# FibonacciDude/ContrastiveProsthetics

Measured on AMD Instinct MI355X. Metric: sEMG windows/sec contrastive step, 12-ch Ninapro, 1/2/4/8 MI355X, higher is better.
Workload: dtype bf16; 1 GPU; synthetic 12-ch sEMG, 41-class one-hot, batch 4096 groups/GPU (167936 windows/GPU/step), stock BN (--no_adabn), dp_emg=0.0635, d_e=16, random-init weights; global_batch_groups=4096, parallelism=dp1, loss=reference per-group loss, tile_schedule=static

## Files before the change

contrastiveprosthetics_amd/_lib.py:

```python
from __future__ import annotations

import ctypes as C
import os

_HERE = os.path.dirname(os.path.abspath(__file__))
LIB_PATH = os.environ.get("CPNATIVE_LIB") or os.path.join(_HERE, "libcpnative.so")

CP_F32, CP_BF16, CP_FP8 = 0, 1, 2
FP8_STATE_BYTES = 1024
CP_TASKS, CP_EMG_DIM, CP_D_E, CP_N_BN, CP_N_FC = 41, 12, 16, 9, 7

_fp = C.c_void_p


class cp_params(C.Structure):
    _fields_ = [
        ("conv1_w", _fp), ("conv1_b", _fp), ("conv2_w", _fp), ("conv2_b", _fp),
        ("fc_w", _fp * CP_N_FC), ("fc_b", _fp * CP_N_FC),
        ("bn_g", _fp * CP_N_BN), ("bn_b", _fp * CP_N_BN),
        ("last_w", _fp), ("easy_w", _fp), ("easy_b", _fp),
    ]


class cp_bn_buffers(C.Structure):
    _fields_ = [("running_mean", _fp * CP_N_BN), ("running_var", _fp * CP_N_BN)]


ALLREDUCE_FN = C.CFUNCTYPE(C.c_int, C.c_void_p, C.c_void_p, C.c_int64, C.c_void_p)

OPTIONS = {"unfused_bn_bwd": 1, "unpaired_wgrad": 2, "fp8_bridge": 4, "no_small": 8, "fp8_head_f32": 16}
CP_TILES_STATIC, CP_TILES_DYNAMIC = 0, 1


class cp_forward_record(C.Structure):
    _fields_ = [("n_windows", C.c_int64), ("path", C.c_int32), ("backwards", C.c_int32), ("transposed", C.c_int32),
                ("pad", C.c_int32), ("join_event", C.c_void_p)]


class cp_config(C.Structure):
    _fields_ = [
        ("n_windows", C.c_int64), ("dtype", C.c_int32), ("adabn", C.c_int32),
        ("training", C.c_int32), ("step_state_lo", C.c_uint32),
        ("dp_emg", C.c_float), ("bn_momentum", C.c_float), ("bn_eps", C.c_float), ("step_state_hi", C.c_uint32),
        ("seed", C.c_uint64), ("step", C.c_uint64),
        ("options", C.c_uint32), ("tile_schedule", C.c_int32),
# ... 327 lines not shown
```

contrastiveprosthetics_amd/csrc/common.cuh:

```cuda
#pragma once
#include <hip/hip_runtime.h>
#include <stdint.h>
#include <type_traits>
#include <utility>

typedef uint16_t bf16_t;
typedef __attribute__((ext_vector_type(8))) short s16x8;
typedef __attribute__((ext_vector_type(4))) short s16x4;
typedef __attribute__((ext_vector_type(4))) float f32x4;
typedef __attribute__((ext_vector_type(16))) float f32x16;

#define CP_WAVE 64

template <class F, int... I>
__device__ __forceinline__ void static_for_impl(F&& f, std::integer_sequence<int, I...>) { (f(std::integral_constant<int, I>{}), ...); }
template <int N, class F>
__device__ __forceinline__ void static_for(F&& f) { static_for_impl(f, std::make_integer_sequence<int, N>{}); }


__device__ __forceinline__ float bf2f(bf16_t h) { return __uint_as_float(((uint32_t)h) << 16); }
__device__ __forceinline__ bf16_t f2bf(float f) {
    return __builtin_bit_cast(bf16_t, (__bf16)f);
}
typedef __bf16 bf16x2_t __attribute__((ext_vector_type(2)));
// ... 175 lines not shown
#pragma unroll
    for (int o = 32; o > 0; o >>= 1) v += __shfl_xor(v, o, 64);
    return v;
}
__device__ __forceinline__ float wave_max(float v) {
#pragma unroll
    for (int o = 32; o > 0; o >>= 1) v = fmaxf(v, __shfl_xor(v, o, 64));
    return v;
}
__device__ __forceinline__ double wave_sum_d(double v) {
#pragma unroll
    for (int o = 32; o > 0; o >>= 1) v += __shfl_xor(v, o, 64);
    return v;
}

static inline int cdiv(int64_t a, int64_t b) { return (int)((a + b - 1) / b); }
```

contrastiveprosthetics_amd/csrc/conv_kernels.cuh:

```cuda
#pragma once
#include <type_traits>
#include "common.cuh"
#include "gemm_tn.cuh"

#define CONV_WPB 16
#define CONV_ROWS (CONV_WPB * 12)
#define CONV_IMG_ROWS (CONV_WPB * 14)

struct ConvArgs {
    const float* x;
    const float* w1;
    const float* b1;
    const float* stats1;
    const void* wc;
    const float* bias2;
    const void* gin;
    const int* gin_exp;
    const float* coef;
    void* out;
    uint8_t* out8;
    const int* out_exp;
    uint32_t* out_amax;
    float* partials;
    int64_t n_windows;
// ... 582 lines not shown

    for (int i = tid; i < 64 * (192 / EPC); i += 256) {
        const int row = i / (192 / EPC), ch = i % (192 / EPC);
        *(uint4*)(Wl + row * WPITCH + ch * 16) = *(const uint4*)((const T*)a.wc + row * 192 + ch * EPC);
    }
    for (int i = tid; i < 2 * CONV_WPB * 16; i += 256) (&xpad[0][0])[i] = 0.f;
    const int ch1 = ft * 32 + r;
    const float w0 = a.w1[ch1 * 9 + 3], w1 = a.w1[ch1 * 9 + 4], w2 = a.w1[ch1 * 9 + 5], b1 = a.b1[ch1];
    float ca, cb, cz;
    if constexpr (ROWS) {
        __shared__ float ca_s[64], cb_s[64], cz_s[64];
        conv_bn_bwd_coef(a.rows1, a.rows1_nr, 1, a.stats1, (double)a.n_windows * 12, ca_s, cb_s, cz_s, (double (*)[4][64])smem, blockIdx.x == 0,
                         a.dgamma1, a.dbeta1);
        ca = ca_s[ch1]; cb = cb_s[ch1]; cz = cz_s[ch1];
        __syncthreads();
    } else {
        ca = a.coef[ch1]; cb = a.coef[64 + ch1]; cz = a.coef[128 + ch1];
    }
    float d0 = 0.f, d1 = 0.f, d2 = 0.f, d3 = 0.f;

    auto load_x = [&](int64_t strip) {
        const int64_t i = strip * (CONV_WPB * 12) + tid;
        return (tid < CONV_WPB * 12 && strip < nstrips && i < total_rows) ? a.x[i] : 0.f;
    };
    const int xslot = (tid / 12) * 16 + 1 + tid % 12;
    constexpr int NITG = CONV_IMG_ROWS / RPP;
    GV pg[NITG];
    float gd = 1.f;
    if constexpr (G8) gd = f8_exp2i(-*a.gin_exp);
    auto prefetch_g = [&](int64_t strip) {
// ... 100 lines not shown
```

contrastiveprosthetics_amd/csrc/encoder_api.cuh:

```cuda
static const int kLayerC[CP_N_BN] = {64, 64, 512, 512, 512, 512, 512, 512, 512};
static inline int fcK(int i) { return i == 0 ? 768 : 512; }
static inline size_t align256(size_t x) { return (x + 255) & ~(size_t)255; }

struct WS {
    size_t act[CP_N_BN];
    size_t u[4];
    size_t gbuf[2];
    size_t dz;
    size_t partials;
    size_t partials2;
    size_t stats[CP_N_BN];
    size_t coef;
    size_t wc2_f, wc2_d;
    size_t wfc[CP_N_FC], bfc[CP_N_FC], wfc_t[CP_N_FC];
    size_t wlast, blast, wlast_t, dzsum;
    size_t slabs;
    size_t praw;
    size_t head_part;
    size_t sm_acc;
    size_t sync_loc, sync_glob;
    size_t gkeep[3], slabs_b;
    size_t f8state, act8[CP_N_BN], u8[3], wfc8[CP_N_FC], wsc8[CP_N_FC];
    size_t g8[2], wfc8t[CP_N_FC], wsc8t[CP_N_FC];
    size_t total;
// ... 160 lines not shown
static inline int grid_rows(int64_t rows, int rows_per_block, int cap) {
    int64_t g = (rows + rows_per_block - 1) / rows_per_block;
    return (int)(g > cap ? cap : (g < 1 ? 1 : g));
}

template <typename T> static inline int fc_bm() { return sizeof(T) == 2 ? 256 : 128; }
template <typename T, int EPI>
static inline hipError_t launch_fc_gemm(const GemmNTArgs& a, hipStream_t st, int* stat_rows = nullptr, bool dyn_schedule = false) {
    if (stat_rows) *stat_rows = (int)((a.M + fc_bm<T>() - 1) / fc_bm<T>());
    if constexpr (sizeof(T) == 2) {
        const bool dyn = dyn_schedule, ws_ok = !dyn;
        if (EPI == EPI_FWD && a.K == WS_K && a.lda == WS_K && a.relu && ws_ok) return launch_gemm_ws(a, st, stat_rows);
        if (EPI == EPI_FWD && a.K == WSK_K && a.lda == WSK_K && a.F == 512 && a.relu && ws_ok) return launch_gemm_ws16n(a, st, stat_rows);
        if (EPI == EPI_FWD || (a.R == nullptr && a.dp_thresh == 0)) return launch_gemm_nt256p<EPI>(a, st, stat_rows, dyn);
        if (EPI == EPI_DGRAD && a.R != nullptr && a.K == WS_K && a.lda == WS_K && ws_ok) return launch_gemm_wsd_bn(a, st, stat_rows);
        if constexpr (EPI == EPI_DGRAD)
            return a.coef ? launch_gemm_nt256p<EPI_DGRAD_BN>(a, st, stat_rows, dyn) : launch_gemm_nt256p<EPI_DGRAD_ST>(a, st, stat_rows, dyn);
        return hipErrorInvalidValue;
    } else {
        return launch_gemm_nt<T, 128, 128, ALOAD_PLAIN, EPI>(a, st);
    }
}

template <typename T>
static inline int conv_grid(int64_t n_windows) {
    const int64_t strips = (n_windows + CONV_WPB - 1) / CONV_WPB;
    const int64_t cap = sizeof(T) == 2 ? 512 : 256;
    return (int)(strips < cap ? strips : cap);
}

// ... 482 lines not shown

static int bwd_finalize(const Pass& ctx, cp_params* g, const float* pp, int nr, double count, int l, int C, int nfold, const char* what) {
    const cp_config* c = ctx.cfg;
    const float* local = nullptr;
    if (c->stats_allreduce) {
        if (int e = sync_row(c, pp, nr, 2 * C * nfold, ctx.base, ctx.w, ctx.st, &pp, &local)) return e;
        nr = 1;
        count *= c->stats_world;
    }
    hipLaunchKernelGGL(bn_bwd_finalize_kernel, dim3(FIN_GRID(C)), dim3(FIN_THREADS), 0, ctx.st, pp, nr, count, ctx.stats(l), ctx.coef, g->bn_g[l],
                       g->bn_b[l], C, nfold, local);
    CKL(what);
    return 0;
}

static int bias_grad_from_rows(const Pass& ctx, int rows, int C, float* db, const char* what) {
    const float* pp = ctx.pre(rows, C);
    hipLaunchKernelGGL(colsum_finalize_kernel, dim3(FIN_GRID(C)), dim3(FIN_THREADS), 0, ctx.st, pp, rows, C, db);
    CKL(what);
    return 0;
}

template <typename T>
static int proj_dz_sums(const ProjLaunch& ctx, const T* dz, float* dzsum) {
    using D = DT<T>;
    const int gb = grid_rows(ctx.N, 256 / (CP_D_E / D::EPC), 64);
    hipLaunchKernelGGL((colsum_kernel<T>), dim3(gb), dim3(256), 256 * D::EPC * 4, ctx.st, dz, ctx.partials, ctx.N, 64, CP_D_E);
    hipLaunchKernelGGL(colsum_finalize_kernel, dim3(FIN_GRID(CP_D_E)), dim3(FIN_THREADS), 0, ctx.st, ctx.partials, gb, CP_D_E, dzsum);
    CKL("colsum(dz)");
    return 0;
// ... 194 lines not shown
    if (!small && gcol_rows <= 0) {
        if (int e = launch_conv2_gcols<T>(ctx.conv(), cur, &gcol_rows)) return e;
    }
    ConvArgs ca{};
    ca.x = x; ca.w1 = p->conv1_w; ca.b1 = p->conv1_b; ca.stats1 = nullptr; ca.gin = cur; ca.n_windows = N;
    if (small) {
        float* gcols3 = (float*)(base + w.praw);
        ca.bn2_rows = partials; ca.bn2_nr = stat_rows; ca.r2 = ctx.act<T>(1); ca.stats2 = ctx.stats(1);
        ca.dgamma2 = g->bn_g[1]; ca.dbeta2 = g->bn_b[1]; ca.gcols3 = gcols3;
        if (int e = conv2_wgrad<T>(ctx.conv(), p, g, ca, true, false, nullptr, 0, gcols3, g->conv2_b)) return e;
        if (int e = tap_gradient(c, 1, cur, N, 768, sizeof(T), st)) return e;
    } else {
        ca.gin_exp = g8 ? (const int*)&g8->e[F8_T_GRAD + 1] : nullptr;
        if (int e = conv2_wgrad<T>(ctx.conv(), p, g, ca, false, g8 != nullptr, partials, gcol_rows, nullptr, nullptr)) return e;
        ProfScope ps(CP_K_BN_BWD, st);
        if (int e = bwd_finalize(ctx, g, ctx.rows2(), CONV2_FINISH_ROWS, (double)R12, 0, 64, 1, "bn_bwd_finalize_kernel(conv1)")) return e;
        ca.coef = ctx.coef;
    }
    int grid_d = 0;
    ca.wc = base + w.wc2_d;
    if (c->grad_tap) {
        ca.out = nxt; ca.partials = partials;
        if (g8) ca.gin = (unsigned char*)c->grad_tap + (size_t)N * 768 * 2;
        if (int e = launch_conv2_dgrad<T>(ctx.conv(), ca, &grid_d)) return e;
        ca.gin = cur;
        if (int e = tap_gradient(c, 0, nxt, N, 768, sizeof(T), st)) return e;
    }
    {
        ca.out = nullptr; ca.partials = partials;
        if (small) {
            ca.stats1 = ctx.stats(0); ca.rows1 = ctx.rows2(); ca.rows1_nr = CONV2_FINISH_ROWS;
            ca.dgamma1 = g->bn_g[0]; ca.dbeta1 = g->bn_b[0];
// ... 98 lines not shown
    if (int e = aux.fork()) return e;
    {
        ProfScope ps(CP_K_PROJ_BWD, st);
        const ProjLaunch pl = ctx.proj();
        const float *s = nullptr, *t = nullptr;
        float* dzsum = (float*)(base + w.dzsum);
        if (!drop) {
            s = ctx.scale(8); t = ctx.shift(8);
            if (int e = proj_dz_sums<T>(pl, dz, dzsum)) return e;
        }
        ProjDrop dp{};
        if (drop) set_dropout(dp, ctx, 8);
        const hipStream_t sw = aux.s();
        int S;
        const bool proj_alg = fuse_ok && drop && sizeof(T) == 2;
        if (proj_alg) {
            if constexpr (sizeof(T) == 2) {
                if (int e = launch_proj_wgrad_onepass(pl, (const bf16_t*)dz, ctx.act<T>(8), nullptr, slabs, dp, ctx.scale(8), ctx.shift(8), p->last_w, g->last_w, &S)) return e;
            }
        } else {
            if (int e = launch_proj_wgrad_tn<T>(pl, sw, dz, ctx.act<T>(8), nullptr, aux.on ? (float*)(base + w.slabs_b) : slabs, ctx.scale(8), ctx.shift(8), dp,
                                                s, t, dzsum, g->last_w, drop ? (float*)nullptr : praw, &S)) return e;
        }
        if (!drop) {
            if (int e = proj_sums_from_wgrad(pl, p->last_w, praw, dzsum)) return e;
            stat_rows = 1;
        }
        GemmNTArgs a{};
        a.A = dz; a.lda = 64; a.M = N; a.K = 64;
        a.W = base + w.wlast_t; a.F = 512;
        a.C = cur; a.ldc = 512; a.R = drop ? ctx.act<T>(8) : nullptr; a.ldr = 512; a.partials = partials;
        if (drop) set_dropout(a, ctx, 8);
        int drows = 0;
        if (fuse_ok && !drop) {
            if (int e = bwd_finalize(ctx, g, partials, stat_rows, (double)N, 8, 512, 1, "bn_bwd_finalize_kernel(fc7, fused)")) return e;
            a.R = ctx.act<T>(8); a.coef = coef; a.coef_mod = 512;
            CK((launch_fc_gemm<T, EPI_DGRAD>(a, st, &drows, dyn_tiles(c))));
            if (int e = bias_grad_from_rows(ctx, drows, 512, g->fc_b[6], "colsum_finalize_kernel(fc7, fused)")) return e;
            bn_done = true;
        } else if (proj_alg) {
            if (int e = bwd_finalize(ctx, g, partials, PROJ_FINISH_ROWS, (double)N, 8, 512, 1, "bn_bwd_finalize_kernel(fc7, projection)")) return e;
            a.coef = coef; a.coef_mod = 512;
            CK(launch_proj_dgrad(a, st, &drows));
            if (int e = bias_grad_from_rows(ctx, drows, 512, g->fc_b[6], "colsum_finalize_kernel(fc7, projection)")) return e;
            bn_done = true;
        } else {
            CK((launch_fc_gemm<T, EPI_DGRAD>(a, st, &drows, dyn_tiles(c))));
            if (drop) stat_rows = drows;
        }
    }
    struct { const T* X; const T* Y; int i; } pend{};
    bool pending = false;
    for (int L = 8; L >= 2; --L) {
        const int i = L - 2, Lp = L - 1, K = fcK(i);
        if (!bn_done) {
            ProfScope ps(CP_K_BN_BWD, st);
            int nr = stat_rows;
            const float* pp = ctx.pre(nr, 2 * 512);
            if (int e = bwd_finalize(ctx, g, pp, nr, (double)N, L, 512, 1, "bn_bwd_finalize_kernel")) return e;
            const int gb = grid_rows(N, 256 / (512 / D::EPC), CAP_BRB16);
            hipLaunchKernelGGL((bn_relu_bwd_kernel<T>), dim3(gb), dim3(256), 256 * D::EPC * 4, st, cur, ctx.act<T>(L), coef, partials, N, 512);
            if (int e = bias_grad_from_rows(ctx, gb, 512, g->fc_b[i], "bn_relu_bwd_kernel")) return e;
        }
        if (int e = tap_gradient(c, L, cur, N, 512, sizeof(T), st)) return e;
        const bool in_drop = drop && Lp >= 5;
        const T* Y = in_drop ? (const T*)(base + w.u[Lp - 5]) : ctx.act<T>(Lp);
        const float* s = in_drop ? nullptr : ctx.scale(Lp);
        const float* t = in_drop ? nullptr : ctx.shift(Lp);
        int S;
        WgradPlace pl;
        if (int e = place_wgrad(ctx, aux, in_drop, i, sizeof(T) == 2 && !opt(c, CP_OPT_UNPAIRED_WGRAD), &pl)) return e;
        if (pl.defer) {
            pend.X = cur; pend.Y = Y; pend.i = i;
            pending = true;
        } else if constexpr (sizeof(T) == 2) {
            GemmTN256Args ta{};
            ta.X = (const bf16_t*)cur; ta.ldx = 512; ta.Y = (const bf16_t*)Y; ta.ldy = K; ta.slabs = pl.slabs; ta.M = N; ta.P = 512; ta.Q = K;
            if (pending) { ta.X2 = (const bf16_t*)pend.X; ta.Y2 = (const bf16_t*)pend.Y; ta.slabs2 = pl.slabs + (size_t)32 * 512 * 512; }
            split_rows(N, pending ? 32 : (K == 512 ? 64 : 40), &S, &ta.rows_per_split);
            ta.splits = S;
            ProfScope ps(CP_K_FC_WGRAD, pl.sw);
            CK(launch_gemm_tn256(ta, pl.sw));
        } else {
            GemmTNArgs ta{};
            ta.X = cur; ta.ldx = 512; ta.Y = Y; ta.ldy = K; ta.slabs = slabs; ta.M = N; ta.P = 512; ta.Q = K;
            split_rows(N, 32, &S, &ta.rows_per_split);
            ProfScope ps(CP_K_FC_WGRAD, st);
            CK((launch_gemm_tn<T, 128, 128, YLOAD_PLAIN>(ta, S, st)));
        }
        if (!pl.defer) {
            ProfScope ps(CP_K_REDUCE_SLABS, pl.sw);
            if (pending) {
                hipLaunchKernelGGL(reduce_slabs_kernel<float>, dim3(512), dim3(256), 0, pl.sw, pl.slabs + (size_t)32 * 512 * 512, S, 512, 512, 512,
                                   (const float*)nullptr, (const float*)nullptr, g->fc_b[pend.i], g->fc_w[pend.i], 0, (float*)nullptr);
                CKL("reduce_slabs(fc, deferred)");
                pending = false;
            }
            hipLaunchKernelGGL(reduce_slabs_kernel<float>, dim3(512), dim3(256), 0, pl.sw, pl.slabs, S, 512, K, 512, s, t, g->fc_b[i], g->fc_w[i],
                               i == 0 ? 1 : 0, in_drop ? (float*)nullptr : praw);
            CKL("reduce_slabs(fc)");
            if (!in_drop) {
                hipLaunchKernelGGL(bn_bwd_sums_from_wgrad_kernel, dim3(K / 64, kSumSlices), dim3(256), 0, st, praw, p->fc_w[i],
                                   g->fc_b[i], partials, 512, K, i == 0 ? 1 : 0);
                CKL("bn_bwd_sums_from_wgrad_kernel");
            }
        }
        stat_rows = in_drop ? tiles_n : kSumSlices;
        GemmNTArgs a{};
        a.A = cur; a.lda = 512; a.M = N; a.K = 512;
        a.W = base + w.wfc_t[i]; a.F = K;
        a.C = nxt; a.ldc = K; a.R = in_drop ? ctx.act<T>(Lp) : nullptr; a.ldr = K; a.partials = partials;
        if (in_drop) set_dropout(a, ctx, Lp);
        bn_done = false;
        if (fuse_ok && !in_drop) {
            const int Cp = kLayerC[Lp], nfold = K / Cp;
            {
                ProfScope ps(CP_K_BN_BWD, st);
                int nr = stat_rows;
                const float* pp = ctx.pre(nr, 2 * K);
                if (int e = bwd_finalize(ctx, g, pp, nr, (double)N * nfold, Lp, Cp, nfold, "bn_bwd_finalize_kernel(fused)")) return e;
            }
            a.R = ctx.act<T>(Lp); a.coef = coef; a.coef_mod = Cp;
            int drows = 0;
            {
                ProfScope ps(CP_K_FC_DGRAD_BN, st);
                CK((launch_fc_gemm<T, EPI_DGRAD>(a, st, &drows, dyn_tiles(c))));
            }
            if (Lp == 1) gcol_rows = drows;
            {
                ProfScope ps(CP_K_BN_BWD, st);
                if (int e = bias_grad_from_rows(ctx, drows * nfold, Cp, Lp >= 2 ? g->fc_b[i - 1] : g->conv2_b, "colsum_finalize_kernel(fused)")) return e;
            }
            bn_done = true;
        } else {
            ProfScope ps(in_drop ? CP_K_FC_DGRAD_STATS : CP_K_FC_DGRAD, st);
// ... 272 lines not shown
```

contrastiveprosthetics_amd/csrc/gemm_nt.cuh:

```cuda
#pragma once
#include "common.cuh"

enum { ALOAD_PLAIN = 0, ALOAD_CONV = 1,
       ALOAD_BNDROP = 2,
       ALOAD_F8 = 3,
       ALOAD_BNDROP_F8 = 4 };
enum { EPI_FWD = 0, EPI_DGRAD = 1, EPI_PLAIN_F32 = 2,
       EPI_DGRAD_BN = 3,
       EPI_DGRAD_ST = 4 };

struct GemmNTArgs {
    const void* A;
    const void* W;
    void* C;
    const float* bias;
    const void* R;
    float* partials;
    const float* coef;
    int coef_mod;
    const float* a_scale;
    const float* a_shift;
    const int* a_exp;
    int64_t M;
    int lda, ldc, ldr;
    int K, F;
    int relu;
    int f_valid;
    int pad0;
    uint32_t dp_thresh, dp_key;
    const uint32_t* dp_salt;
    float dp_inv_keep;
    int* sched;
};

template <typename T, int BM, int BN, int ALOAD, int EPI>
__global__ __launch_bounds__(256) void gemm_nt_kernel(GemmNTArgs a) {
    using D = DT<T>;
    constexpr int EPC = D::EPC;
    constexpr int BK = D::BK;
    constexpr int WAVES_F = (BN >= 128) ? 2 : 1;
    constexpr int WAVES_S = 4 / WAVES_F;
    constexpr int WS_T = BM / (WAVES_S * 32);
    constexpr int WF_T = BN / (WAVES_F * 32);
    constexpr int A_BYTES = BM * 128, W_BYTES = BN * 128;
    constexpr int C_PITCH = BN * (int)sizeof(T) + 16;
    constexpr int STAGE_BYTES = 2 * (A_BYTES + W_BYTES);
    constexpr int C_BYTES = (EPI == EPI_PLAIN_F32) ? 0 : BM * C_PITCH;
// ... 225 lines not shown
```

contrastiveprosthetics_amd/csrc/gemm_ws.cuh:

```cuda
#pragma once
#include "gemm_nt256p.cuh"

#define WS_K 512

template <typename V4, typename RSRC>
__device__ __forceinline__ void store_b128_settled(const V4& c, RSRC rsrc, uint32_t voff, uint32_t soff, int ) {
    __builtin_amdgcn_raw_buffer_store_b128(c, rsrc, voff, soff, 0);
    asm volatile("s_nop 1" :: "v"(c));
}

typedef __attribute__((ext_vector_type(4))) unsigned int u32x4_t;
__device__ __forceinline__ void bufl16_lds(const u32x4_t& rsrc, uint32_t voff, uint32_t soff_uniform, uint32_t lds_dst_uniform) {
    uint32_t keep;
    asm volatile("s_mov_b32 %0, m0\n\ts_mov_b32 m0, %4\n\ts_nop 0\n\tbuffer_load_dwordx4 %1, %2, %3 offen lds\n\ts_mov_b32 m0, %0"
                 : "=&s"(keep)
                 : "v"(voff), "s"(rsrc), "s"(soff_uniform), "s"(lds_dst_uniform)
                 : "memory");
}

typedef __attribute__((ext_vector_type(4))) float f32x4_t;
#define WS16_RT 48
#define WS16_ST (WS16_RT / 16)
#define WS16_TILE_BYTES (WS16_RT * WS_K * 2)
struct Ws16Acc {
// ... 359 lines not shown
    if (stat_rows) *stat_rows = (int)(tiles < workers ? tiles : workers);
    if (a.partials != nullptr) hipLaunchKernelGGL(gemm_ws16n_kernel<true>, dim3(256), dim3(256), 0, st, a);
    else hipLaunchKernelGGL(gemm_ws16n_kernel<false>, dim3(256), dim3(256), 0, st, a);
    return hipGetLastError();
}


#define WSD16_RT 32

template <int MODE>
__global__ __launch_bounds__(256, 1) void gemm_wsd16_kernel(GemmNTArgs a) {
    constexpr bool STATS = MODE == 1;
    constexpr int RT = WSD16_RT, TILE_BYTES = RT * WS_K * 2, R_BYTES = RT * 128;
    constexpr int K = WS_K, KB = K / 32, RPW = RT / 4, ST = RT / 16;
    constexpr int R_OFF = 2 * TILE_BYTES, COEF_OFF = R_OFF + 4 * 2 * R_BYTES;
    __shared__ __attribute__((aligned(16))) unsigned char smem[COEF_OFF];

    const int tid = threadIdx.x, lane = tid & 63;
    const int wave = __builtin_amdgcn_readfirstlane(tid >> 6);
    const int s16 = lane & 15, q4 = lane >> 4;
    const int xcd = blockIdx.x & 7, j = blockIdx.x >> 3;
    const int nfb = a.F >> 8;
    const int nwk = 32 / nfb;
    const int fb = j % nfb, wkr = j / nfb;
    const int64_t tiles = (a.M + RT - 1) / RT;
    const int first = wkr * 8 + xcd, stride = nwk * 8;
    const int ntile = (wkr < nwk && first < tiles) ? (int)((tiles - first + stride - 1) / stride) : 0;
    if (ntile == 0) return;
    const uint32_t dkey = (STATS && a.dp_thresh != 0) ? (a.dp_salt ? (a.dp_key ^ *a.dp_salt) : a.dp_key) : 0u;
    const int f0 = fb * 256 + wave * 64;
    float4 cfa[STATS ? 1 : 4], cfb[STATS ? 1 : 4], cfz[STATS ? 1 : 4];
    if constexpr (!STATS) {
#pragma unroll
        for (int ft = 0; ft < 4; ++ft) {
            float v[3][4];
#pragma unroll
            for (int c = 0; c < 3; ++c)
#pragma unroll
                for (int e = 0; e < 4; ++e) v[c][e] = a.coef[c * a.coef_mod + (f0 + ft * 16 + 4 * (lane >> 4) + e) % a.coef_mod];
            cfa[ft] = make_float4(v[0][0], v[0][1], v[0][2], v[0][3]);
            cfb[ft] = make_float4(v[1][0], v[1][1], v[1][2], v[1][3]);
            cfz[ft] = make_float4(v[2][0], v[2][1], v[2][2], v[2][3]);
        }
    }

    s16x8 wreg[4][KB];
    {
        const bf16_t* Wg = (const bf16_t*)a.W + (int64_t)(f0 + s16) * K + 8 * q4;
#pragma unroll
        for (int ft = 0; ft < 4; ++ft)
#pragma unroll
            for (int kb = 0; kb < KB; ++kb)
                asm volatile("global_load_dwordx4 %0, %1, off" : "=a"(wreg[ft][kb]) : "v"(Wg + (int64_t)ft * 16 * K + kb * 32) : "memory");
        asm volatile("s_waitcnt vmcnt(0)" ::: "memory");
#pragma unroll
        for (int ft = 0; ft < 4; ++ft)
#pragma unroll
            for (int kb = 0; kb < KB; kb += 8)
                asm volatile("s_waitcnt vmcnt(0)" : "+a"(wreg[ft][kb]), "+a"(wreg[ft][kb + 1]), "+a"(wreg[ft][kb + 2]), "+a"(wreg[ft][kb + 3]),
                             "+a"(wreg[ft][kb + 4]), "+a"(wreg[ft][kb + 5]), "+a"(wreg[ft][kb + 6]), "+a"(wreg[ft][kb + 7]));
// ... 168 lines not shown
    constexpr int COEF_OFF = 4 * 2 * R_BYTES;
    __shared__ __attribute__((aligned(16))) unsigned char smem[COEF_OFF + 3 * 256 * 4];
    float* coef_s = (float*)(smem + COEF_OFF);

    const int tid = threadIdx.x, lane = tid & 63;
    const int wave = __builtin_amdgcn_readfirstlane(tid >> 6);
    const int s16 = lane & 15, q4 = lane >> 4;
    const int xcd = blockIdx.x & 7, j = blockIdx.x >> 3;
    const int nfb = a.F >> 8;
    const int nwk = (gridDim.x >> 3) / nfb;
    const int fb = j % nfb, wkr = j / nfb;
    const int64_t tiles = (a.M + RT - 1) / RT;
    const int first = wkr * 8 + xcd, stride = nwk * 8;
    const int ntile = (wkr < nwk && first < tiles) ? (int)((tiles - first + stride - 1) / stride) : 0;
    if (ntile == 0) return;
    for (int q = tid; q < 3 * 256; q += 256) {
        const int c = q >> 8, f = fb * 256 + (q & 255);
        coef_s[q] = a.coef[c * a.coef_mod + f % a.coef_mod];
    }
    __syncthreads();
    const int f0 = fb * 256 + wave * 64, fl0 = wave * 64;
    const uint32_t dkey = a.dp_thresh != 0 ? (a.dp_salt ? (a.dp_key ^ *a.dp_salt) : a.dp_key) : 0u;

    typedef short s16x4_t __attribute__((ext_vector_type(4)));
    s16x4_t wfrag[4];
#pragma unroll
    for (int ft = 0; ft < 4; ++ft) wfrag[ft] = *(const s16x4_t*)((const bf16_t*)a.W + (int64_t)(f0 + ft * 16 + s16) * a.K + 4 * q4);

    const uint32_t lds0 = __builtin_amdgcn_readfirstlane((uint32_t)(uintptr_t)smem);
    const uint64_t r_base = (uint64_t)(uintptr_t)a.R;
    const u32x4_t r_rsrc = {(uint32_t)r_base, (uint32_t)(r_base >> 32) & 0xFFFFu, (uint32_t)(a.M * a.ldr * 2), 0x00020000u};
    const uint32_t r_lane = (uint32_t)((lane >> 3) * a.ldr * 2 + f0 * 2);
    auto fetch_r = [&](int64_t m0, int buf) {
// ... 88 lines not shown
#pragma unroll
        for (int st = 0; st < ST; ++st) dzf[st] = dzn[st];
    }
    if (s16 < 8) {
        const int64_t prow = (int64_t)wkr * 8 + xcd;
#pragma unroll
        for (int fp = 0; fp < 2; ++fp) {
            const int f = f0 + fp * 32 + (s16 >> 2) * 16 + 4 * q4 + (s16 & 3);
            a.partials[prow * a.F + f] = qs1[fp];
        }
    }
}

static inline hipError_t launch_proj_dgrad(const GemmNTArgs& a, hipStream_t st, int* stat_rows) {
    if ((a.F & 255) || a.K < 16 || (a.K & 3) || !a.R || !a.coef) return hipErrorInvalidValue;
#define PROJ_DGRAD_BLOCKS 512
    const int blocks = PROJ_DGRAD_BLOCKS, nwk = (blocks >> 3) / (a.F >> 8);
    const int64_t tiles = (a.M + PROJ_RT - 1) / PROJ_RT, workers = (int64_t)nwk * 8;
    if (stat_rows) *stat_rows = (int)(tiles < workers ? tiles : workers);
    hipLaunchKernelGGL(proj_dgrad_kernel, dim3(blocks), dim3(256), 0, st, a);
    return hipGetLastError();
}

static inline hipError_t launch_gemm_wsd_bn(const GemmNTArgs& a, hipStream_t st, int* stat_rows) {
    if (a.K != WS_K || (a.F & 255) || a.F > 768 || a.lda != WS_K || !a.R) return hipErrorInvalidValue;
    const int nfb = a.F >> 8, nwk = 32 / nfb;
    const int64_t tiles = (a.M + WSD16_RT - 1) / WSD16_RT;
    const int64_t workers = (int64_t)nwk * 8;
    if (stat_rows) *stat_rows = (int)(tiles < workers ? tiles : workers);
    if (!a.coef) hipLaunchKernelGGL(gemm_wsd16_kernel<1>, dim3(256), dim3(256), 0, st, a);
    else hipLaunchKernelGGL(gemm_wsd16_kernel<0>, dim3(256), dim3(256), 0, st, a);
    return hipGetLastError();
}

static inline hipError_t launch_gemm_ws(const GemmNTArgs& a, hipStream_t st, int* stat_rows) {
    if (a.K != WS_K || (a.F & 255) || a.F > 768 || a.lda != WS_K) return hipErrorInvalidValue;
    const int nfb = a.F >> 8, nwk = 32 / nfb;
    const int64_t tiles = (a.M + WS16_RT - 1) / WS16_RT;
    const int64_t workers = (int64_t)nwk * 8;
    if (stat_rows) *stat_rows = (int)(tiles < workers ? tiles : workers);
// ... 5 lines not shown
```

contrastiveprosthetics_amd/csrc/kernels_misc.cuh:

```cuda
#pragma once
#include "common.cuh"

__device__ unsigned int g_gather_oob;
__global__ void gather_groups_kernel(const float* __restrict__ table, const int64_t* __restrict__ emg_rand,
                                     const int64_t* __restrict__ perm, float* __restrict__ out, int64_t B, int T,
                                     int V, int64_t D, int64_t table_rows) {
    const int64_t total = B * T * V * 3;
    for (int64_t i = blockIdx.x * (int64_t)blockDim.x + threadIdx.x; i < total; i += (int64_t)gridDim.x * blockDim.x) {
        const int q = (int)(i % 3);
        const int64_t win = i / 3;
        const int v = (int)(win % V);
        const int64_t bt = win / V;
        const int t = (int)(bt % T);
        const int64_t b = bt / T;
        int64_t src = emg_rand[(int64_t)t * D + perm[b]] * V + v;
        if (src < 0 || src >= table_rows) {
            if (q == 0) atomicAdd(&g_gather_oob, 1u);
            src = 0;
        }
        *(float4*)(out + win * 12 + q * 4) = *(const float4*)(table + src * 12 + q * 4);
    }
}

#define AUG_NORM_C 0x1.bb67aep-16f
// ... 509 lines not shown
#pragma unroll
        for (int u = 0; u < 8; ++u) v[u] = partials[((int64_t)(r + u) * 4 + k) * 64 + c];
#pragma unroll
        for (int u = 0; u < 8; ++u) s += (double)v[u];
    }
    for (; r < nrows; ++r) s += (double)partials[((int64_t)r * 4 + k) * 64 + c];
    if (k < 3) {
        dW[c * 9 + 3 + k] = (float)s;
        dW[c * 9 + 0 + k] = 0.f;
        dW[c * 9 + 6 + k] = 0.f;
    } else {
        db[c] = (float)s;
    }
}

template <typename ST = float>
__global__ void reduce_slabs_kernel(const float* __restrict__ slabs_, int S, int P, int Q, int p_valid,
                                    const float* __restrict__ s, const float* __restrict__ t,
                                    const float* __restrict__ dbsum, float* __restrict__ grad, int mode,
                                    float* __restrict__ raw, const int* __restrict__ exp_x = nullptr, const int* __restrict__ exp_y = nullptr) {
    const float unscale = exp_x != nullptr ? f8_exp2i(-*exp_x - *exp_y) : 1.f;
    const int64_t total4 = (int64_t)p_valid * Q / 4;
    const int64_t sstride = (int64_t)P * Q;
    for (int64_t i4 = blockIdx.x * (int64_t)blockDim.x + threadIdx.x; i4 < total4; i4 += (int64_t)gridDim.x * blockDim.x) {
        const int64_t i = i4 * 4;
        const int p = (int)(i / Q), q0 = (int)(i % Q);
        const ST* src = (const ST*)slabs_ + (int64_t)p * Q + q0;
        auto ld = [&](int kk, float (&v)[4]) {
            if constexpr (sizeof(ST) == 2) {
                const uint2 w = *(const uint2*)(src + kk * sstride);
                v[0] = __uint_as_float(w.x << 16); v[1] = __uint_as_float(w.x & 0xffff0000u);
                v[2] = __uint_as_float(w.y << 16); v[3] = __uint_as_float(w.y & 0xffff0000u);
            } else {
                const float4 w = *(const float4*)(src + kk * sstride);
                v[0] = w.x; v[1] = w.y; v[2] = w.z; v[3] = w.w;
// ... 18 lines not shown
            for (int e = 0; e < 4; ++e) a[0][e] += v0[e];
        }
#pragma unroll
        for (int e = 0; e < 4; ++e) {
            const int q = q0 + e;
            float acc = ((a[0][e] + a[1][e]) + (a[2][e] + a[3][e])) * unscale;
            if (raw != nullptr) raw[i + e] = acc;
            int ch = q, dst = p * Q + q;
            if (mode == 1) { ch = q & 63; dst = p * Q + ch * 12 + (q >> 6); }
            if (mode == 3) dst = q * p_valid + p;
            if (s != nullptr) acc = fmaf(s[ch], acc, t[ch] * dbsum[p]);
            grad[dst] = acc;
        }
    }
}

#define CONV2_FINISH_ROWS 64
template <typename T>
__global__ __launch_bounds__(256) void conv2_wgrad_finish_kernel(const float* __restrict__ slabs, int S, const float* __restrict__ gcols, int nr,
                                                                 const float* __restrict__ W2, const float* __restrict__ stats1,
                                                                 float* __restrict__ dW2, float* __restrict__ out_rows,
                                                                 const float* __restrict__ gcols3 = nullptr, float* __restrict__ db2 = nullptr) {
    using D = DT<T>;
    __shared__ double part[21][12];
    __shared__ float Gs[3];
    __shared__ float red[2][3][64];
    const int tid = threadIdx.x, o = blockIdx.x;
    const int ncol = gcols3 ? 3 : 12;
    if (tid < 21 * ncol) {
        const int q = tid % ncol, ls = tid / ncol;
// ... 77 lines not shown
```

include/cpnative.h:

```cpp
#ifndef CPNATIVE_H
#define CPNATIVE_H

#include <stddef.h>
#include <stdint.h>

#ifdef __cplusplus
extern "C" {
#endif

#define CP_VERSION 112
#define CP_F32 0
#define CP_BF16 1
#define CP_FP8 2
#define CP_TASKS 41
#define CP_EMG_DIM 12
#define CP_D_E 16
#define CP_N_BN 9
#define CP_N_FC 7
#define CP_ERR_ARG 10001
#define CP_ERR_WORKSPACE 10002

typedef struct cp_params {
    float* conv1_w;
    float* conv1_b;
// ... 8 lines not shown
    float* easy_b;
} cp_params;

typedef struct cp_bn_buffers {
    float* running_mean[CP_N_BN];
    float* running_var[CP_N_BN];
} cp_bn_buffers;

typedef int (*cp_allreduce_fn)(void* user, void* row_dev, int64_t count, void* stream);

#define CP_OPT_UNFUSED_BN_BWD 1u
#define CP_OPT_UNPAIRED_WGRAD 2u
#define CP_OPT_FP8_BRIDGE 4u
#define CP_OPT_NO_SMALL 8u
#define CP_OPT_FP8_HEAD_F32 16u

enum { CP_TILES_STATIC = 0, CP_TILES_DYNAMIC = 1 };

typedef struct cp_forward_record {
    int64_t n_windows;
    int32_t path;
    int32_t backwards;
    int32_t transposed;
    int32_t pad;
    void* join_event;
} cp_forward_record;

typedef struct cp_config {
    int64_t n_windows;
    int32_t dtype;
// ... 559 lines not shown
```

Baseline: 47.93 million windows/s.

## Fold BN backward finalize into consumer kernel prologues and pair slab reductions

Instead of launching a separate bn_bwd_finalize kernel for conv1, the projection and the fused FC layers, each consumer kernel (conv dgrad, proj dgrad, wsd_bn gemm) now reduces the partial-sum rows and computes the BN coefficients in its own prologue. Only one block writes dgamma/dbeta. The deferred and current reduce_slabs launches are also merged into one two-job kernel. This removes several small launches and serialization points, but every block now recomputes the coefficient reduction redundantly. A new option flag restores the old path.

```diff
diff --git a/contrastiveprosthetics_amd/_lib.py b/contrastiveprosthetics_amd/_lib.py
--- a/contrastiveprosthetics_amd/_lib.py
+++ b/contrastiveprosthetics_amd/_lib.py
@@ -28,7 +28,8 @@
 
 ALLREDUCE_FN = C.CFUNCTYPE(C.c_int, C.c_void_p, C.c_void_p, C.c_int64, C.c_void_p)
 
-OPTIONS = {"unfused_bn_bwd": 1, "unpaired_wgrad": 2, "fp8_bridge": 4, "no_small": 8, "fp8_head_f32": 16}
+OPTIONS = {"unfused_bn_bwd": 1, "unpaired_wgrad": 2, "fp8_bridge": 4, "no_small": 8, "fp8_head_f32": 16,
+           "finalize_launches": 32}
 CP_TILES_STATIC, CP_TILES_DYNAMIC = 0, 1
 
 
diff --git a/contrastiveprosthetics_amd/csrc/common.cuh b/contrastiveprosthetics_amd/csrc/common.cuh
--- a/contrastiveprosthetics_amd/csrc/common.cuh
+++ b/contrastiveprosthetics_amd/csrc/common.cuh
@@ -213,4 +213,52 @@
     return v;
 }
 
+#define BNP_MAX_ROWS 64
+template <int NFOLD>
+struct BnpQuad { float v1[4][NFOLD], v2[4][NFOLD]; };
+template <int NFOLD>
+__device__ __forceinline__ void bnp_load(BnpQuad<NFOLD>& u, const float* __restrict__ rows, int nr, int C, int c, int q) {
+    const int W = C * NFOLD;
+#pragma unroll
+    for (int gi = 0; gi < 4; ++gi) {
+        const int r = 4 * q + gi;
+        const bool ok = r < nr;
+        const float* p = rows + (int64_t)(ok ? r : 0) * 2 * W + c;
+#pragma unroll
+        for (int f = 0; f < NFOLD; ++f) {
+            const float a = p[f * C], b = p[W + f * C];
+            u.v1[gi][f] = ok ? a : 0.f;
+            u.v2[gi][f] = ok ? b : 0.f;
+        }
+    }
+}
+template <int NFOLD>
+__device__ __forceinline__ void bnp_quad_sum(const BnpQuad<NFOLD>& u, double& w1, double& w2) {
+    double s1[4], s2[4];
+#pragma unroll
+    for (int gi = 0; gi < 4; ++gi) {
+        s1[gi] = s2[gi] = 0;
+#pragma unroll
+        for (int f = 0; f < NFOLD; ++f) { s1[gi] += (double)u.v1[gi][f]; s2[gi] += (double)u.v2[gi][f]; }
+    }
+    w1 = (s1[0] + s1[1]) + (s1[2] + s1[3]);
+    w2 = (s2[0] + s2[1]) + (s2[2] + s2[3]);
+}
+__device__ __forceinline__ double bnp_total(const double* w, int nq, int stride) {
+    double t = 0;
+    for (int q = 0; q < nq; ++q) t += w[q * stride];
+    return t;
+}
+__device__ __forceinline__ void bnp_coef(double s1, double s2, const float* __restrict__ stats, int C, int c, double count, float& ca, float& cb,
+                                         float& cz, float& dgamma, float& dbeta) {
+    const double mean = stats[c], invstd = stats[C + c], sc = stats[2 * C + c];
+    const double dot = (s2 - mean * s1) * invstd;
+    const double c1 = s1 / count, c2 = dot / count;
+    ca = (float)sc;
+    cb = (float)(-sc * invstd * c2);
+    cz = (float)(-sc * (c1 - mean * invstd * c2));
+    dgamma = (float)dot;
+    dbeta = (float)s1;
+}
+
 static inline int cdiv(int64_t a, int64_t b) { return (int)((a + b - 1) / b); }
diff --git a/contrastiveprosthetics_amd/csrc/conv_kernels.cuh b/contrastiveprosthetics_amd/csrc/conv_kernels.cuh
--- a/contrastiveprosthetics_amd/csrc/conv_kernels.cuh
+++ b/contrastiveprosthetics_amd/csrc/conv_kernels.cuh
@@ -620,6 +620,30 @@
                          a.dgamma1, a.dbeta1);
         ca = ca_s[ch1]; cb = cb_s[ch1]; cz = cz_s[ch1];
         __syncthreads();
+    } else if (a.rows1 != nullptr) {
+        __shared__ float cf_s[3][64];
+        static_assert(IMG_BYTES >= 2 * 16 * 64 * 8, "the quads' sums use the image region");
+        double* quad_s = (double*)smem;
+        const int c = tid & 63, part = tid >> 6;
+        BnpQuad<1> bq[4];
+#pragma unroll
+        for (int i = 0; i < 4; ++i) bnp_load(bq[i], a.rows1, a.rows1_nr, 64, c, part + 4 * i);
+#pragma unroll
+        for (int i = 0; i < 4; ++i) {
+            double w1, w2;
+            bnp_quad_sum(bq[i], w1, w2);
+            quad_s[(part + 4 * i) * 64 + c] = w1;
+            quad_s[(16 + part + 4 * i) * 64 + c] = w2;
+        }
+        __syncthreads();
+        if (tid < 64) {
+            float dg, db;
+            bnp_coef(bnp_total(quad_s + c, 16, 64), bnp_total(quad_s + 16 * 64 + c, 16, 64), a.stats1, 64, c, (double)a.n_windows * 12, cf_s[0][c], cf_s[1][c],
+                     cf_s[2][c], dg, db);
+            if (blockIdx.x == 0) { a.dgamma1[c] = dg; a.dbeta1[c] = db; }
+        }
+        __syncthreads();
+        ca = cf_s[0][ch1]; cb = cf_s[1][ch1]; cz = cf_s[2][ch1];
     } else {
         ca = a.coef[ch1]; cb = a.coef[64 + ch1]; cz = a.coef[128 + ch1];
     }
diff --git a/contrastiveprosthetics_amd/csrc/encoder_api.cuh b/contrastiveprosthetics_amd/csrc/encoder_api.cuh
--- a/contrastiveprosthetics_amd/csrc/encoder_api.cuh
+++ b/contrastiveprosthetics_amd/csrc/encoder_api.cuh
@@ -198,6 +198,7 @@
         if (EPI == EPI_FWD && a.K == WSK_K && a.lda == WSK_K && a.F == 512 && a.relu && ws_ok) return launch_gemm_ws16n(a, st, stat_rows);
         if (EPI == EPI_FWD || (a.R == nullptr && a.dp_thresh == 0)) return launch_gemm_nt256p<EPI>(a, st, stat_rows, dyn);
         if (EPI == EPI_DGRAD && a.R != nullptr && a.K == WS_K && a.lda == WS_K && ws_ok) return launch_gemm_wsd_bn(a, st, stat_rows);
+        if (a.bn_rows) return hipErrorInvalidValue;
         if constexpr (EPI == EPI_DGRAD)
             return a.coef ? launch_gemm_nt256p<EPI_DGRAD_BN>(a, st, stat_rows, dyn) : launch_gemm_nt256p<EPI_DGRAD_ST>(a, st, stat_rows, dyn);
         return hipErrorInvalidValue;
@@ -710,6 +711,13 @@
     return 0;
 }
 
+static inline bool bwd_in_prologue(const Pass& ctx, int nr, int max_rows) {
+    return !opt(ctx.cfg, CP_OPT_FINALIZE_LAUNCHES) && !ctx.cfg->stats_allreduce && nr <= max_rows;
+}
+static inline void set_bn_prologue(GemmNTArgs& a, const Pass& ctx, cp_params* g, const float* rows, int nr, double count, int l) {
+    a.bn_rows = rows; a.bn_nr = nr; a.bn_stats = ctx.stats(l); a.bn_count = count; a.bn_dgamma = g->bn_g[l]; a.bn_dbeta = g->bn_b[l];
+}
+
 static int bias_grad_from_rows(const Pass& ctx, int rows, int C, float* db, const char* what) {
     const float* pp = ctx.pre(rows, C);
     hipLaunchKernelGGL(colsum_finalize_kernel, dim3(FIN_GRID(C)), dim3(FIN_THREADS), 0, ctx.st, pp, rows, C, db);
@@ -934,8 +942,13 @@
         ca.gin_exp = g8 ? (const int*)&g8->e[F8_T_GRAD + 1] : nullptr;
         if (int e = conv2_wgrad<T>(ctx.conv(), p, g, ca, false, g8 != nullptr, partials, gcol_rows, nullptr, nullptr)) return e;
         ProfScope ps(CP_K_BN_BWD, st);
-        if (int e = bwd_finalize(ctx, g, ctx.rows2(), CONV2_FINISH_ROWS, (double)R12, 0, 64, 1, "bn_bwd_finalize_kernel(conv1)")) return e;
-        ca.coef = ctx.coef;
+        if (!g8 && bwd_in_prologue(ctx, CONV2_FINISH_ROWS, BNP_MAX_ROWS)) {
+            ca.stats1 = ctx.stats(0); ca.rows1 = ctx.rows2(); ca.rows1_nr = CONV2_FINISH_ROWS;
+            ca.dgamma1 = g->bn_g[0]; ca.dbeta1 = g->bn_b[0];
+        } else {
+            if (int e = bwd_finalize(ctx, g, ctx.rows2(), CONV2_FINISH_ROWS, (double)R12, 0, 64, 1, "bn_bwd_finalize_kernel(conv1)")) return e;
+            ca.coef = ctx.coef;
+        }
     }
     int grid_d = 0;
     ca.wc = base + w.wc2_d;
@@ -1064,9 +1077,12 @@
         const hipStream_t sw = aux.s();
         int S;
         const bool proj_alg = fuse_ok && drop && sizeof(T) == 2;
+        const bool proj_pro = proj_alg && bwd_in_prologue(ctx, PROJ_FINISH_ROWS, 16);
         if (proj_alg) {
             if constexpr (sizeof(T) == 2) {
-                if (int e = launch_proj_wgrad_onepass(pl, (const bf16_t*)dz, ctx.act<T>(8), nullptr, slabs, dp, ctx.scale(8), ctx.shift(8), p->last_w, g->last_w, &S)) return e;
+                ProjLaunch pw = pl;
+                if (proj_pro) pw.partials = ctx.rows2();
+                if (int e = launch_proj_wgrad_onepass(pw, (const bf16_t*)dz, ctx.act<T>(8), nullptr, slabs, dp, ctx.scale(8), ctx.shift(8), p->last_w, g->last_w, &S)) return e;
             }
         } else {
             if (int e = launch_proj_wgrad_tn<T>(pl, sw, dz, ctx.act<T>(8), nullptr, aux.on ? (float*)(base + w.slabs_b) : slabs, ctx.scale(8), ctx.shift(8), dp,
@@ -1089,7 +1105,8 @@
             if (int e = bias_grad_from_rows(ctx, drows, 512, g->fc_b[6], "colsum_finalize_kernel(fc7, fused)")) return e;
             bn_done = true;
         } else if (proj_alg) {
-            if (int e = bwd_finalize(ctx, g, partials, PROJ_FINISH_ROWS, (double)N, 8, 512, 1, "bn_bwd_finalize_kernel(fc7, projection)")) return e;
+            if (proj_pro) set_bn_prologue(a, ctx, g, ctx.rows2(), PROJ_FINISH_ROWS, (double)N, 8);
+            else if (int e = bwd_finalize(ctx, g, partials, PROJ_FINISH_ROWS, (double)N, 8, 512, 1, "bn_bwd_finalize_kernel(fc7, projection)")) return e;
             a.coef = coef; a.coef_mod = 512;
             CK(launch_proj_dgrad(a, st, &drows));
             if (int e = bias_grad_from_rows(ctx, drows, 512, g->fc_b[6], "colsum_finalize_kernel(fc7, projection)")) return e;
@@ -1117,6 +1134,7 @@
         const T* Y = in_drop ? (const T*)(base + w.u[Lp - 5]) : ctx.act<T>(Lp);
         const float* s = in_drop ? nullptr : ctx.scale(Lp);
         const float* t = in_drop ? nullptr : ctx.shift(Lp);
+        const bool dgrad_pro = fuse_ok && !in_drop && !dyn_tiles(c) && bwd_in_prologue(ctx, kSumSlices, 16);
         int S;
         WgradPlace pl;
         if (int e = place_wgrad(ctx, aux, in_drop, i, sizeof(T) == 2 && !opt(c, CP_OPT_UNPAIRED_WGRAD), &pl)) return e;
@@ -1140,18 +1158,27 @@
         }
         if (!pl.defer) {
             ProfScope ps(CP_K_REDUCE_SLABS, pl.sw);
-            if (pending) {
-                hipLaunchKernelGGL(reduce_slabs_kernel<float>, dim3(512), dim3(256), 0, pl.sw, pl.slabs + (size_t)32 * 512 * 512, S, 512, 512, 512,
-                                   (const float*)nullptr, (const float*)nullptr, g->fc_b[pend.i], g->fc_w[pend.i], 0, (float*)nullptr);
-                CKL("reduce_slabs(fc, deferred)");
+            if (pending && !opt(c, CP_OPT_FINALIZE_LAUNCHES)) {
+                ReduceSlabsPair rp{};
+                rp.job[0] = ReduceSlabsJob{pl.slabs + (size_t)32 * 512 * 512, nullptr, nullptr, g->fc_b[pend.i], g->fc_w[pend.i], nullptr, S, 512, 512, 512, 0};
+                rp.job[1] = ReduceSlabsJob{pl.slabs, s, t, g->fc_b[i], g->fc_w[i], in_drop ? (float*)nullptr : praw, S, 512, K, 512, i == 0 ? 1 : 0};
+                hipLaunchKernelGGL(reduce_slabs_pair_kernel, dim3(512, 2), dim3(256), 0, pl.sw, rp);
+                CKL("reduce_slabs_pair(fc)");
                 pending = false;
+            } else {
+                if (pending) {
+                    hipLaunchKernelGGL(reduce_slabs_kernel<float>, dim3(512), dim3(256), 0, pl.sw, pl.slabs + (size_t)32 * 512 * 512, S, 512, 512, 512,
+                                       (const float*)nullptr, (const float*)nullptr, g->fc_b[pend.i], g->fc_w[pend.i], 0, (float*)nullptr);
+                    CKL("reduce_slabs(fc, deferred)");
+                    pending = false;
+                }
+                hipLaunchKernelGGL(reduce_slabs_kernel<float>, dim3(512), dim3(256), 0, pl.sw, pl.slabs, S, 512, K, 512, s, t, g->fc_b[i], g->fc_w[i],
+                                   i == 0 ? 1 : 0, in_drop ? (float*)nullptr : praw);
+                CKL("reduce_slabs(fc)");
             }
-            hipLaunchKernelGGL(reduce_slabs_kernel<float>, dim3(512), dim3(256), 0, pl.sw, pl.slabs, S, 512, K, 512, s, t, g->fc_b[i], g->fc_w[i],
-                               i == 0 ? 1 : 0, in_drop ? (float*)nullptr : praw);
-            CKL("reduce_slabs(fc)");
             if (!in_drop) {
                 hipLaunchKernelGGL(bn_bwd_sums_from_wgrad_kernel, dim3(K / 64, kSumSlices), dim3(256), 0, st, praw, p->fc_w[i],
-                                   g->fc_b[i], partials, 512, K, i == 0 ? 1 : 0);
+                                   g->fc_b[i], dgrad_pro ? ctx.rows2() : partials, 512, K, i == 0 ? 1 : 0);
                 CKL("bn_bwd_sums_from_wgrad_kernel");
             }
         }
@@ -1168,7 +1195,8 @@
                 ProfScope ps(CP_K_BN_BWD, st);
                 int nr = stat_rows;
                 const float* pp = ctx.pre(nr, 2 * K);
-                if (int e = bwd_finalize(ctx, g, pp, nr, (double)N * nfold, Lp, Cp, nfold, "bn_bwd_finalize_kernel(fused)")) return e;
+                if (dgrad_pro) set_bn_prologue(a, ctx, g, ctx.rows2(), nr, (double)N * nfold, Lp);
+                else if (int e = bwd_finalize(ctx, g, pp, nr, (double)N * nfold, Lp, Cp, nfold, "bn_bwd_finalize_kernel(fused)")) return e;
             }
             a.R = ctx.act<T>(Lp); a.coef = coef; a.coef_mod = Cp;
             int drows = 0;
diff --git a/contrastiveprosthetics_amd/csrc/gemm_nt.cuh b/contrastiveprosthetics_amd/csrc/gemm_nt.cuh
--- a/contrastiveprosthetics_amd/csrc/gemm_nt.cuh
+++ b/contrastiveprosthetics_amd/csrc/gemm_nt.cuh
@@ -31,6 +31,12 @@
     const uint32_t* dp_salt;
     float dp_inv_keep;
     int* sched;
+    const float* bn_rows;
+    const float* bn_stats;
+    float* bn_dgamma;
+    float* bn_dbeta;
+    double bn_count;
+    int bn_nr;
 };
 
 template <typename T, int BM, int BN, int ALOAD, int EPI>
diff --git a/contrastiveprosthetics_amd/csrc/gemm_ws.cuh b/contrastiveprosthetics_amd/csrc/gemm_ws.cuh
--- a/contrastiveprosthetics_amd/csrc/gemm_ws.cuh
+++ b/contrastiveprosthetics_amd/csrc/gemm_ws.cuh
@@ -397,7 +397,8 @@
     constexpr int RT = WSD16_RT, TILE_BYTES = RT * WS_K * 2, R_BYTES = RT * 128;
     constexpr int K = WS_K, KB = K / 32, RPW = RT / 4, ST = RT / 16;
     constexpr int R_OFF = 2 * TILE_BYTES, COEF_OFF = R_OFF + 4 * 2 * R_BYTES;
-    __shared__ __attribute__((aligned(16))) unsigned char smem[COEF_OFF];
+    constexpr int BNP_BYTES = STATS ? 0 : 3 * 256 * 4 + 2 * 4 * 64 * 8;
+    __shared__ __attribute__((aligned(16))) unsigned char smem[COEF_OFF + BNP_BYTES];
 
     const int tid = threadIdx.x, lane = tid & 63;
     const int wave = __builtin_amdgcn_readfirstlane(tid >> 6);
@@ -413,20 +414,67 @@
     const uint32_t dkey = (STATS && a.dp_thresh != 0) ? (a.dp_salt ? (a.dp_key ^ *a.dp_salt) : a.dp_key) : 0u;
     const int f0 = fb * 256 + wave * 64;
     float4 cfa[STATS ? 1 : 4], cfb[STATS ? 1 : 4], cfz[STATS ? 1 : 4];
+    const bool bnp = !STATS && a.bn_rows != nullptr, bnp_wide = a.coef_mod == a.F;
     if constexpr (!STATS) {
-#pragma unroll
-        for (int ft = 0; ft < 4; ++ft) {
-            float v[3][4];
-#pragma unroll
-            for (int c = 0; c < 3; ++c)
-#pragma unroll
-                for (int e = 0; e < 4; ++e) v[c][e] = a.coef[c * a.coef_mod + (f0 + ft * 16 + 4 * (lane >> 4) + e) % a.coef_mod];
-            cfa[ft] = make_float4(v[0][0], v[0][1], v[0][2], v[0][3]);
-            cfb[ft] = make_float4(v[1][0], v[1][1], v[1][2], v[1][3]);
-            cfz[ft] = make_float4(v[2][0], v[2][1], v[2][2], v[2][3]);
-        }
-    }
-
+        if (!bnp) {
+#pragma unroll
+            for (int ft = 0; ft < 4; ++ft) {
+                float v[3][4];
+#pragma unroll
+                for (int c = 0; c < 3; ++c)
+#pragma unroll
+                    for (int e = 0; e < 4; ++e) v[c][e] = a.coef[c * a.coef_mod + (f0 + ft * 16 + 4 * (lane >> 4) + e) % a.coef_mod];
+                cfa[ft] = make_float4(v[0][0], v[0][1], v[0][2], v[0][3]);
+                cfb[ft] = make_float4(v[1][0], v[1][1], v[1][2], v[1][3]);
+                cfz[ft] = make_float4(v[2][0], v[2][1], v[2][2], v[2][3]);
+            }
+        }
+    }
+
+    if constexpr (!STATS) {
+        if (bnp) {
+            float* coef_s = (float*)(smem + COEF_OFF);
+            double* quad_s = (double*)(smem + COEF_OFF + 3 * 256 * 4);
+            const bool writer = xcd == 0 && wkr == 0;
+            if (bnp_wide) {
+                const int c = fb * 256 + tid;
+                double w1[4], w2[4];
+#pragma unroll
+                for (int q = 0; q < 4; ++q) {
+                    BnpQuad<1> bq;
+                    bnp_load(bq, a.bn_rows, a.bn_nr, a.F, c, q);
+                    bnp_quad_sum(bq, w1[q], w2[q]);
+                }
+                float ca, cb, cz, dg, db;
+                bnp_coef(bnp_total(w1, 4, 1), bnp_total(w2, 4, 1), a.bn_stats, a.F, c, a.bn_count, ca, cb, cz, dg, db);
+                coef_s[tid] = ca; coef_s[256 + tid] = cb; coef_s[512 + tid] = cz;
+                if (writer) { a.bn_dgamma[c] = dg; a.bn_dbeta[c] = db; }
+            } else {
+                const int c = tid & 63, q = tid >> 6;
+                BnpQuad<12> bq;
+                bnp_load(bq, a.bn_rows, a.bn_nr, 64, c, q);
+                double w1, w2;
+                bnp_quad_sum(bq, w1, w2);
+                quad_s[q * 64 + c] = w1;
+                quad_s[(4 + q) * 64 + c] = w2;
+                __syncthreads();
+                if (tid < 64) {
+                    float ca, cb, cz, dg, db;
+                    bnp_coef(bnp_total(quad_s + c, 4, 64), bnp_total(quad_s + 4 * 64 + c, 4, 64), a.bn_stats, 64, c, a.bn_count, ca, cb, cz, dg, db);
+                    coef_s[c] = ca; coef_s[256 + c] = cb; coef_s[512 + c] = cz;
+                    if (writer && fb == 0) { a.bn_dgamma[c] = dg; a.bn_dbeta[c] = db; }
+                }
+            }
+            __syncthreads();
+            const int fl = (bnp_wide ? wave * 64 : 0) + 4 * q4;
+#pragma unroll
+            for (int ft = 0; ft < 4; ++ft) {
+                cfa[ft] = *(const float4*)(coef_s + fl + ft * 16);
+                cfb[ft] = *(const float4*)(coef_s + 256 + fl + ft * 16);
+                cfz[ft] = *(const float4*)(coef_s + 512 + fl + ft * 16);
+            }
+        }
+    }
     s16x8 wreg[4][KB];
     {
         const bf16_t* Wg = (const bf16_t*)a.W + (int64_t)(f0 + s16) * K + 8 * q4;
@@ -625,9 +673,23 @@
     const int first = wkr * 8 + xcd, stride = nwk * 8;
     const int ntile = (wkr < nwk && first < tiles) ? (int)((tiles - first + stride - 1) / stride) : 0;
     if (ntile == 0) return;
-    for (int q = tid; q < 3 * 256; q += 256) {
-        const int c = q >> 8, f = fb * 256 + (q & 255);
-        coef_s[q] = a.coef[c * a.coef_mod + f % a.coef_mod];
+    if (a.bn_rows != nullptr) {
+        BnpQuad<1> bq[4];
+#pragma unroll
+        for (int q = 0; q < 4; ++q) bnp_load(bq[q], a.bn_rows, a.bn_nr, a.F, fb * 256 + tid, q);
+        double w1[4], w2[4];
+#pragma unroll
+        for (int q = 0; q < 4; ++q) bnp_quad_sum(bq[q], w1[q], w2[q]);
+        const int c = fb * 256 + tid;
+        float ca, cb, cz, dg, db;
+        bnp_coef(bnp_total(w1, 4, 1), bnp_total(w2, 4, 1), a.bn_stats, a.F, c, a.bn_count, ca, cb, cz, dg, db);
+        coef_s[tid] = ca; coef_s[256 + tid] = cb; coef_s[512 + tid] = cz;
+        if (xcd == 0 && wkr == 0) { a.bn_dgamma[c] = dg; a.bn_dbeta[c] = db; }
+    } else {
+        for (int q = tid; q < 3 * 256; q += 256) {
+            const int c = q >> 8, f = fb * 256 + (q & 255);
+            coef_s[q] = a.coef[c * a.coef_mod + f % a.coef_mod];
+        }
     }
     __syncthreads();
     const int f0 = fb * 256 + wave * 64, fl0 = wave * 64;
@@ -746,6 +808,7 @@
 
 static inline hipError_t launch_proj_dgrad(const GemmNTArgs& a, hipStream_t st, int* stat_rows) {
     if ((a.F & 255) || a.K < 16 || (a.K & 3) || !a.R || !a.coef) return hipErrorInvalidValue;
+    if (a.bn_rows && (a.coef_mod != a.F || a.bn_nr < 1 || a.bn_nr > 16 || !a.bn_stats || !a.bn_dgamma || !a.bn_dbeta)) return hipErrorInvalidValue;
 #define PROJ_DGRAD_BLOCKS 512
     const int blocks = PROJ_DGRAD_BLOCKS, nwk = (blocks >> 3) / (a.F >> 8);
     const int64_t tiles = (a.M + PROJ_RT - 1) / PROJ_RT, workers = (int64_t)nwk * 8;
@@ -756,6 +819,9 @@
 
 static inline hipError_t launch_gemm_wsd_bn(const GemmNTArgs& a, hipStream_t st, int* stat_rows) {
     if (a.K != WS_K || (a.F & 255) || a.F > 768 || a.lda != WS_K || !a.R) return hipErrorInvalidValue;
+    if (a.bn_rows && (!a.coef || !(a.coef_mod == a.F || (a.coef_mod == 64 && a.F == 768)) || a.bn_nr < 1 || a.bn_nr > 16 || !a.bn_stats ||
+                      !a.bn_dgamma || !a.bn_dbeta))
+        return hipErrorInvalidValue;
     const int nfb = a.F >> 8, nwk = 32 / nfb;
     const int64_t tiles = (a.M + WSD16_RT - 1) / WSD16_RT;
     const int64_t workers = (int64_t)nwk * 8;
diff --git a/contrastiveprosthetics_amd/csrc/kernels_misc.cuh b/contrastiveprosthetics_amd/csrc/kernels_misc.cuh
--- a/contrastiveprosthetics_amd/csrc/kernels_misc.cuh
+++ b/contrastiveprosthetics_amd/csrc/kernels_misc.cuh
@@ -547,11 +547,11 @@
     }
 }
 
-template <typename ST = float>
-__global__ void reduce_slabs_kernel(const float* __restrict__ slabs_, int S, int P, int Q, int p_valid,
-                                    const float* __restrict__ s, const float* __restrict__ t,
-                                    const float* __restrict__ dbsum, float* __restrict__ grad, int mode,
-                                    float* __restrict__ raw, const int* __restrict__ exp_x = nullptr, const int* __restrict__ exp_y = nullptr) {
+template <typename ST>
+__device__ __forceinline__ void reduce_slabs_body(const float* __restrict__ slabs_, int S, int P, int Q, int p_valid,
+                                                  const float* __restrict__ s, const float* __restrict__ t,
+                                                  const float* __restrict__ dbsum, float* __restrict__ grad, int mode,
+                                                  float* __restrict__ raw, const int* __restrict__ exp_x, const int* __restrict__ exp_y) {
     const float unscale = exp_x != nullptr ? f8_exp2i(-*exp_x - *exp_y) : 1.f;
     const int64_t total4 = (int64_t)p_valid * Q / 4;
     const int64_t sstride = (int64_t)P * Q;
@@ -600,6 +600,19 @@
         }
     }
 }
+template <typename ST = float>
+__global__ void reduce_slabs_kernel(const float* __restrict__ slabs_, int S, int P, int Q, int p_valid,
+                                    const float* __restrict__ s, const float* __restrict__ t,
+                                    const float* __restrict__ dbsum, float* __restrict__ grad, int mode,
+                                    float* __restrict__ raw, const int* __restrict__ exp_x = nullptr, const int* __restrict__ exp_y = nullptr) {
+    reduce_slabs_body<ST>(slabs_, S, P, Q, p_valid, s, t, dbsum, grad, mode, raw, exp_x, exp_y);
+}
+struct ReduceSlabsJob { const float* slabs; const float* s; const float* t; const float* dbsum; float* grad; float* raw; int S, P, Q, p_valid, mode; };
+struct ReduceSlabsPair { ReduceSlabsJob job[2]; };
+__global__ void reduce_slabs_pair_kernel(ReduceSlabsPair rp) {
+    const ReduceSlabsJob& j = rp.job[blockIdx.y];
+    reduce_slabs_body<float>(j.slabs, j.S, j.P, j.Q, j.p_valid, j.s, j.t, j.dbsum, j.grad, j.mode, j.raw, nullptr, nullptr);
+}
 
 #define CONV2_FINISH_ROWS 64
 template <typename T>
diff --git a/include/cpnative.h b/include/cpnative.h
--- a/include/cpnative.h
+++ b/include/cpnative.h
@@ -46,6 +46,7 @@
 #define CP_OPT_FP8_BRIDGE 4u
 #define CP_OPT_NO_SMALL 8u
 #define CP_OPT_FP8_HEAD_F32 16u
+#define CP_OPT_FINALIZE_LAUNCHES 32u
 
 enum { CP_TILES_STATIC = 0, CP_TILES_DYNAMIC = 1 };
 
```

After: 48.50 million windows/s (median of 6 runs). 1.01x the previous value.
